# bacpop/Pansim

Measured on AMD Instinct MI355X. Metric: generations/sec, higher is better.
Workload: dtype u8

## Files before the change

pansim_amd/csrc/acc_kernels.h:

```cpp
#pragma once

#include "ps_common.h"

struct acc_dims { uint32_t N, G, W, GW; };

__global__ void acc_init_kernel(uint64_t *accG, uint64_t *accI, const uint8_t *init_vec, acc_dims d)
{
    const uint64_t t = (uint64_t)blockIdx.x * blockDim.x + threadIdx.x;
    const uint64_t nG = (uint64_t)d.G * d.W, nI = (uint64_t)d.N * d.GW;
    if (t < nG) {
        const uint32_t g = (uint32_t)(t / d.W), w = (uint32_t)(t % d.W);
        const uint32_t nb = min(64u, d.N - w * 64u);
        const uint64_t m = (nb == 64u) ? ~0ull : ((1ull << nb) - 1ull);
        accG[t] = init_vec[g] ? m : 0ull;
    } else if (t < nG + nI) {
        const uint64_t u = t - nG;
        const uint32_t gw = (uint32_t)(u % d.GW);
        uint64_t word = 0;
        for (uint32_t b = 0; b < 64; b++) {
            const uint32_t g = gw * 64u + b;
            if (g < d.G && init_vec[g]) word |= 1ull << b;
        }
        accI[u] = word;
    }
// ... 75 lines not shown
            const ps_u4 r = ps_philox(gw * 16u + j, i, a.gen, PS_STREAM_ACC_MUT, a.k0, a.k1);
            const uint4 t = thr[j];
            const uint32_t b = 4u * j;
            lt[b >> 5] |= ((r.x < t.x ? 1u : 0u) | (r.y < t.y ? 2u : 0u) | (r.z < t.z ? 4u : 0u) | (r.w < t.w ? 8u : 0u)) << (b & 31u);
        }
        word ^= ((uint64_t)lt[1] << 32) | lt[0];
    } else if (DO_MUT) {
        const uint32_t t0 = a.plan.n_comp > 0 ? a.plan.flip_thr[0] : 0u, t1 = a.plan.n_comp > 1 ? a.plan.flip_thr[1] : 0u;
        const uint64_t m0 = a.plan.n_comp > 0 ? ps_word_range_mask(gw, a.plan.comp_begin[0], a.plan.comp_end[0]) : 0ull;
        const uint64_t m1 = a.plan.n_comp > 1 ? ps_word_range_mask(gw, a.plan.comp_begin[1], a.plan.comp_end[1]) : 0ull;
        uint32_t lt0[2] = { 0u, 0u }, lt1[2] = { 0u, 0u };
#pragma unroll
        for (uint32_t j = 0; j < 16u; j++) {
            const ps_u4 r = ps_philox(gw * 16u + j, i, a.gen, PS_STREAM_ACC_MUT, a.k0, a.k1);
            const uint32_t w[4] = { r.x, r.y, r.z, r.w };
#pragma unroll
            for (uint32_t k = 0; k < 4u; k++) {
                const uint32_t b = 4u * j + k;
                lt0[b >> 5] |= (w[k] < t0 ? 1u : 0u) << (b & 31u);
                lt1[b >> 5] |= (w[k] < t1 ? 1u : 0u) << (b & 31u);
            }
        }
        const uint64_t f0 = ((uint64_t)lt0[1] << 32) | lt0[0], f1 = ((uint64_t)lt1[1] << 32) | lt1[0];
        word ^= (f1 & m1) | (f0 & m0 & ~m1);
    }
    a.dstI[t] = word;
    if (a.snapI) a.snapI[t] = word;
}

struct acc_hgt_args {
    const uint64_t *srcI;
    uint64_t *dstI;
    acc_dims d;
    uint32_t n_comp;
    uint32_t gb[PS_MAX_COMP], ge[PS_MAX_COMP];
    const uint32_t *ptab[PS_MAX_COMP];
    uint32_t kmin[PS_MAX_COMP], plen[PS_MAX_COMP];
    uint32_t *work_ctr;
    uint32_t gen, k0, k1;
    uint32_t *bins, *counts;
    uint32_t bin_cap;
    uint32_t parts, rows_per_part;
    uint32_t part_magic;
    uint32_t *scratch;
    unsigned long long *ovf_img;
    uint32_t *overflow_flag;
    uint16_t *list_scratch;
    uint32_t list_stride;
    uint32_t dn_lo, dn_cnt;
    uint32_t bin_prio;
    const uint16_t *wq[PS_MAX_COMP];
    const uint64_t *wnz[PS_MAX_COMP];
    uint32_t pref_off;
};

__device__ __forceinline__ uint32_t ps_hgt_count(const acc_hgt_args &a, uint32_t c, uint32_t dn)
{
    if (!a.ptab[c]) return 0u;
    const ps_u4 r = ps_philox(dn, 0u, a.gen, PS_STREAM_HGT_COUNT | (c << 8), a.k0, a.k1);
    uint32_t lo = 0, hi = a.plen[c];
    while (lo < hi) {
        const uint32_t mid = (lo + hi) >> 1;
        if (a.ptab[c][mid] <= r.x) lo = mid + 1u; else hi = mid;
    }
    if (lo >= a.plen[c]) lo = a.plen[c] - 1u;
    return a.kmin[c] + lo;
}

__global__ void __launch_bounds__(256) acc_snapshot_kernel(const uint64_t *copy_src, uint64_t *copy_dst, uint64_t words)
{
    for (uint64_t w = (uint64_t)blockIdx.x * blockDim.x + threadIdx.x; w < words; w += (uint64_t)gridDim.x * blockDim.x)
        copy_dst[w] = copy_src[w];
}

__device__ __forceinline__ uint32_t ps_wave_gene_list(const uint64_t *row, uint32_t GW, uint32_t gb, uint32_t ge,
                                                      uint16_t *list, uint32_t lane)
{
    uint32_t base = 0;
    for (uint32_t gw0 = gb >> 6; gw0 * 64u < ge; gw0 += 64u) {
        const uint32_t gw = gw0 + lane;
        uint64_t word = 0;
        if (gw * 64u < ge && gw < GW) {
            word = row[gw];
            const uint32_t lo = gw * 64u;
            if (lo < gb) word &= ~0ull << (gb - lo);
            if (lo + 64u > ge) word &= (ge - lo >= 64u) ? ~0ull : ((1ull << (ge - lo)) - 1ull);
        }
        const uint32_t pc = __popcll(word);
        uint32_t incl = pc;
        for (int off = 1; off < 64; off <<= 1) {
            const uint32_t t = __shfl_up(incl, off, 64);
            if ((int)lane >= off) incl += t;
        }
        uint32_t pos = base + incl - pc;
        while (word) {
            const uint32_t b = (uint32_t)__builtin_ctzll(word);
            word &= word - 1ull;
            list[pos++] = (uint16_t)(gw * 64u + b);
        }
        base += __shfl(incl, 63, 64);
    }
    return base;
}

__device__ __forceinline__ uint32_t ps_wave_gene_list_w(const uint64_t *row, uint32_t GW, uint32_t G, const uint64_t *wnz, const uint16_t *wq,
                                                        uint16_t *list, uint32_t *pref, uint32_t lane, uint32_t *total)
{
    uint32_t base = 0, wbase = 0;
    for (uint32_t gw0 = 0; gw0 * 64u < G; gw0 += 64u) {
        const uint32_t gw = gw0 + lane;
        uint64_t word = 0;
        if (gw < GW) word = row[gw] & wnz[gw];
        const uint32_t pc = __popcll(word);
        uint32_t ws = 0;
        for (uint64_t t = word; t; t &= t - 1ull) ws += wq[gw * 64u + (uint32_t)__builtin_ctzll(t)];
        uint32_t incl = pc, wincl = ws;
        for (int off = 1; off < 64; off <<= 1) {
            const uint32_t t = __shfl_up(incl, off, 64), u = __shfl_up(wincl, off, 64);
            if ((int)lane >= off) { incl += t; wincl += u; }
        }
        uint32_t pos = base + incl - pc, run = wbase + wincl - ws;
        while (word) {
            const uint32_t g = gw * 64u + (uint32_t)__builtin_ctzll(word);
            word &= word - 1ull;
            run += wq[g];
            list[pos] = (uint16_t)g;
            pref[pos++] = run;
        }
        base += __shfl(incl, 63, 64);
        wbase += __shfl(wincl, 63, 64);
    }
    *total = wbase;
    return base;
}
__device__ __forceinline__ uint32_t ps_weighted_pick(const uint32_t *pref, uint32_t n, uint32_t total, uint32_t word)
{
    const uint32_t x = ps_mulhi(word, total);
    uint32_t lo = 0, hi = n - 1u;
    while (lo < hi) {
        const uint32_t mid = (lo + hi) >> 1;
        if (pref[mid] > x) hi = mid; else lo = mid + 1u;
    }
    return lo;
}

template <bool WT = false>
__global__ void __launch_bounds__(64) acc_hgt_donor_wave_kernel(acc_hgt_args a)
{
    extern __shared__ __attribute__((aligned(16))) uint16_t lds_list[];
    uint16_t *glist = a.list_scratch ? a.list_scratch + (uint64_t)blockIdx.x * a.list_stride : lds_list;
    uint32_t *pref = (uint32_t *)(glist + a.pref_off);
    uint32_t wtotal = 0;
    const acc_dims d = a.d;
    const uint32_t lane = threadIdx.x;
    const uint32_t items = a.n_comp * a.dn_cnt;
    for (;;) {
        uint32_t item = 0;
        if (lane == 0) item = atomicAdd(a.work_ctr, 1u);
        item = __builtin_amdgcn_readfirstlane(item);
        if (item >= items) break;
        const uint32_t c = item / a.dn_cnt, dn = a.dn_lo + item % a.dn_cnt;
        const uint32_t k = ps_hgt_count(a, c, dn);
        if (k == 0u) continue;
        __threadfence_block();
        const uint32_t n = WT ? ps_wave_gene_list_w(a.srcI + (uint64_t)dn * d.GW, d.GW, d.G, a.wnz[c], a.wq[c], glist, pref, lane, &wtotal)
                              : ps_wave_gene_list(a.srcI + (uint64_t)dn * d.GW, d.GW, a.gb[c], a.ge[c], glist, lane);
        __threadfence_block();
        if (n == 0u) continue;
        const uint32_t stream = PS_STREAM_HGT | (c << 8);
        for (uint32_t jp = lane; 2u * jp < k; jp += 64u) {
            const ps_u4 r = ps_philox(jp, dn, a.gen, stream, a.k0, a.k1);
#pragma unroll
            for (uint32_t h = 0; h < 2u; h++) {
                if (2u * jp + h >= k) break;
                uint32_t rc = ps_mulhi(h ? r.z : r.x, d.N - 1u);
                rc += (rc >= dn) ? 1u : 0u;
                const uint32_t gene = glist[WT ? ps_weighted_pick(pref, n, wtotal, h ? r.w : r.y) : ps_mulhi(h ? r.w : r.y, n)];
                atomicOr((unsigned long long *)&a.dstI[(uint64_t)rc * d.GW + (gene >> 6)], 1ull << (gene & 63u));
            }
        }
    }
}

#ifndef PS_HGT_BIN_BLOCKS
#define PS_HGT_BIN_BLOCKS 2u
#endif
template <bool WT = false>
__global__ void __launch_bounds__(256) acc_hgt_donor_bin_kernel(acc_hgt_args a)
{
    extern __shared__ __attribute__((aligned(16))) uint32_t sc_lds[];
    uint32_t *fill = sc_lds;
    uint16_t *glist = a.list_scratch ? a.list_scratch + (uint64_t)blockIdx.x * a.list_stride
                                     : (uint16_t *)(sc_lds + ((a.parts + 3u) & ~3u));
    __shared__ uint32_t sh_n;
    __shared__ uint32_t sh_total;
    const uint32_t *pref = (const uint32_t *)(glist + a.pref_off);
    const acc_dims d = a.d;
    const uint32_t tid = threadIdx.x, lane = tid & 63u;
    const uint32_t items = a.n_comp * a.dn_cnt;
    const uint32_t cap = a.bin_cap;
    if (a.bin_prio >= 3u) __builtin_amdgcn_s_setprio(3);
    else if (a.bin_prio == 2u) __builtin_amdgcn_s_setprio(2);
    else if (a.bin_prio == 1u) __builtin_amdgcn_s_setprio(1);
    uint32_t *mybins = a.bins + (uint64_t)blockIdx.x * a.parts * cap;
    for (uint32_t q = tid; q < a.parts; q += blockDim.x) fill[q] = 0u;
    for (uint32_t item = blockIdx.x; item < items; item += gridDim.x) {
        __syncthreads();
        const uint32_t c = item / a.dn_cnt, dn = a.dn_lo + item % a.dn_cnt;
        const uint32_t k = ps_hgt_count(a, c, dn);
        if (k == 0u) continue;
        if (tid < 64u) {
            uint32_t tot = 0;
            const uint32_t m = WT ? ps_wave_gene_list_w(a.srcI + (uint64_t)dn * d.GW, d.GW, d.G, a.wnz[c], a.wq[c], glist, (uint32_t *)(glist + a.pref_off), lane, &tot)
                                  : ps_wave_gene_list(a.srcI + (uint64_t)dn * d.GW, d.GW, a.gb[c], a.ge[c], glist, lane);
            if (tid == 0) { sh_n = m; if (WT) sh_total = tot; }
            __threadfence_block();
        }
        __syncthreads();
        const uint32_t n = sh_n;
        if (n == 0u) continue;
        const uint32_t wtotal = WT ? sh_total : 0u;
        const uint32_t stream = PS_STREAM_HGT | (c << 8);
        auto place = [&](uint32_t rc, uint32_t gene, uint32_t part, uint32_t pos) {
            if (pos < cap) mybins[(uint64_t)part * cap + pos] = ((rc - part * a.rows_per_part) << 16) | gene;
            else atomicOr(&a.ovf_img[(uint64_t)rc * d.GW + (gene >> 6)], 1ull << (gene & 63u));
        };
        constexpr uint32_t NBK = PS_HGT_BIN_BLOCKS;
        for (uint32_t jp = tid; 2u * jp < k; jp += NBK * blockDim.x) {
            uint32_t wr[2u * NBK], wg[2u * NBK];
            bool ok[2u * NBK];
#pragma unroll
            for (uint32_t b = 0; b < NBK; b++) {
                const uint32_t jb = jp + b * blockDim.x;
                const ps_u4 r = ps_philox(jb, dn, a.gen, stream, a.k0, a.k1);
                wr[2u * b] = r.x; wg[2u * b] = r.y; wr[2u * b + 1u] = r.z; wg[2u * b + 1u] = r.w;
                ok[2u * b] = 2u * jb < k;
                ok[2u * b + 1u] = 2u * jb + 1u < k;
            }
            uint32_t rc[2u * NBK], gene[2u * NBK], part[2u * NBK], pos[2u * NBK];
#pragma unroll
            for (uint32_t e = 0; e < 2u * NBK; e++) {
                rc[e] = ps_mulhi(wr[e], d.N - 1u);
                rc[e] += (rc[e] >= dn) ? 1u : 0u;
                gene[e] = glist[WT ? ps_weighted_pick(pref, n, wtotal, wg[e]) : ps_mulhi(wg[e], n)];
                part[e] = ps_mulhi(rc[e], a.part_magic);
            }
#pragma unroll
            for (uint32_t e = 0; e < 2u * NBK; e++) pos[e] = ok[e] ? atomicAdd(&fill[part[e]], 1u) : 0u;
#pragma unroll
            for (uint32_t e = 0; e < 2u * NBK; e++)
                if (ok[e]) place(rc[e], gene[e], part[e], pos[e]);
        }
    }
    __syncthreads();
    for (uint32_t q = tid; q < a.parts; q += blockDim.x) {
        a.counts[(uint64_t)blockIdx.x * a.parts + q] = min(fill[q], cap);
    }
}

__global__ void __launch_bounds__(1024) acc_hgt_apply_kernel(acc_hgt_args a, uint32_t donor_blocks, uint32_t n_slices)
{
    extern __shared__ uint32_t lrow[];
// ... 914 lines not shown
```

pansim_amd/csrc/core_kernels.h:

```cpp
#pragma once

#include "ps_common.h"

#include <type_traits>

#define PS_SWEEP_MAX_GENS 2
struct core_sweep_args {
    uint8_t *state;
    uint8_t *out;
    const uint32_t *idx;
    const uint32_t *idx_next[PS_SWEEP_MAX_GENS - 1];
    const uint32_t *idxT;
    uint32_t N, pitch, cpr, rows;
    uint32_t site_offset;
    uint32_t gen, k0, k1;
    ps_core_plan plan;
    uint32_t *overflow_flag;
    unsigned long long *stamps;
    uint32_t *work_ctr;
    uint32_t launch_parity;
    uint32_t nt;
    uint32_t qcap;
    uint32_t qcap_limit;
    uint32_t *wide_flags;
// ... 134 lines not shown
                    const uint32_t k = ps_bit_cell(__builtin_ctz(cm));
                    cm &= cm - 1u;
                    const uint32_t i = c * 16u + k;
                    if (i >= a.N) continue;
                    uint32_t l2y;
                    const ps_cell cell = ps_cell_events<WT>(a, A, B, site, i, a.gen, a.k0, a.k1, pl, l2y);
                    if (DO_MUT && cell.mut) ps_set_byte(d, k, cell.mut);
                    if (DO_HR && cell.hr) hm |= 1u << k;
                }
            }
            if (DO_HR) {
                *(uint4 *)(rowS + 16u * c) = make_uint4(d[0], d[1], d[2], d[3]);
                hrm[c] = (uint16_t)hm;
            } else {
                *(uint4 *)(grow + 16u * c) = make_uint4(d[0], d[1], d[2], d[3]);
            }
        }
        if (DO_HR) {
            __syncthreads();
            for (uint32_t c = lane; c < a.cpr; c += lpr) {
                const uint4 v = *(const uint4 *)(rowS + 16u * c);
                uint32_t d[4] = { v.x, v.y, v.z, v.w };
                uint32_t hm = hrm[c];
                while (hm) {
                    const uint32_t k = __builtin_ctz(hm);
                    hm &= hm - 1u;
                    const uint32_t i = c * 16u + k;
                    const ps_u4 l2 = ps_philox(site, i, a.gen, PS_STREAM_CORE_L2, a.k0, a.k1);
                    uint32_t donor = ps_mulhi(l2.y, a.N - 1u);
                    donor += (donor >= i) ? 1u : 0u;
                    ps_set_byte(d, k, (uint32_t)rowS[donor]);
                }
                *(uint4 *)(grow + 16u * c) = make_uint4(d[0], d[1], d[2], d[3]);
            }
            if (!DO_GATHER) __syncthreads();
        }
    }
}

#define PS_BATCH_ROWS 4u

__device__ __forceinline__ void ps_wave_sync()
{
    __builtin_amdgcn_fence(__ATOMIC_RELEASE, "wavefront");
    __builtin_amdgcn_wave_barrier();
    __builtin_amdgcn_fence(__ATOMIC_ACQUIRE, "wavefront");
}

__device__ __forceinline__ uint32_t ps_lane_prefix(uint64_t bal)
{
    return __builtin_amdgcn_mbcnt_hi((uint32_t)(bal >> 32), __builtin_amdgcn_mbcnt_lo((uint32_t)bal, 0u));
}

__device__ __forceinline__ uint32_t ps_wave_scan_incl(uint32_t x)
{
    x += (uint32_t)__builtin_amdgcn_update_dpp(0, (int)x, 0x111, 0xF, 0xF, false);
    x += (uint32_t)__builtin_amdgcn_update_dpp(0, (int)x, 0x112, 0xF, 0xF, false);
    x += (uint32_t)__builtin_amdgcn_update_dpp(0, (int)x, 0x114, 0xF, 0xF, false);
    x += (uint32_t)__builtin_amdgcn_update_dpp(0, (int)x, 0x118, 0xF, 0xF, false);
    x += (uint32_t)__builtin_amdgcn_update_dpp(0, (int)x, 0x142, 0xA, 0xF, false);
    x += (uint32_t)__builtin_amdgcn_update_dpp(0, (int)x, 0x143, 0xC, 0xF, false);
    return x;
}

struct ps_class_words { uint32_t dec, res; };
__device__ __forceinline__ ps_class_words ps_classes(uint32_t p0, uint32_t p1, uint32_t p2, uint32_t p3, uint32_t p4, uint32_t p5,
                                                     uint32_t k, uint32_t nE, uint32_t vm)
{
    const uint32_t c1 = __builtin_amdgcn_bitop3_b32(p1, p2, p3, 0x01) & vm;
    uint32_t lt;
    switch (nE) {
    case 1: lt = __builtin_amdgcn_bitop3_b32(p0, p5, p4, 0x01); break;
    case 2: lt = __builtin_amdgcn_bitop3_b32(p0, p5, p4, 0x03); break;
    case 3: lt = __builtin_amdgcn_bitop3_b32(p0, p5, p4, 0x07); break;
    case 4: lt = __builtin_amdgcn_bitop3_b32(p0, p5, p4, 0x0F); break;
    case 5: lt = __builtin_amdgcn_bitop3_b32(p0, p5, p4, 0x1F); break;
    case 6: lt = __builtin_amdgcn_bitop3_b32(p0, p5, p4, 0x3F); break;
    case 7: lt = __builtin_amdgcn_bitop3_b32(p0, p5, p4, 0x7F); break;
    default: lt = 0xFFFFFFFFu; break;
    }
    ps_class_words o;
    o.dec = k ? c1 & __builtin_amdgcn_bitop3_b32(p0, p5, p4, 0x07) : 0u;
    o.res = c1 & lt & ~o.dec;
    return o;
}

struct ps_apply_words { uint32_t y0, y1, ya, yb, yc; };
PS_HD uint32_t ps_bfi(uint32_t m, uint32_t a, uint32_t b)
{
#if defined(__HIP_DEVICE_COMPILE__) && __has_builtin(__builtin_amdgcn_bitop3_b32)
    return __builtin_amdgcn_bitop3_b32(m, a, b, 0xCA);
#else
    return (a & m) | (b & ~m);
#endif
}
__device__ __forceinline__ ps_apply_words ps_apply_prepare(uint32_t dec, uint32_t p4, uint32_t p5)
{
    const uint32_t r1 = p5 >> 1, r2 = p4 >> 2, l1 = p5 << 1, l2 = dec << 2;
    ps_apply_words o;
    o.y0 = ps_bfi(0x01010101u, p4, ps_bfi(0x02020202u, l1, l2));
    o.y1 = ps_bfi(0x02020202u, p4, ps_bfi(0x04040404u, l1, l2));
    o.ya = ps_bfi(0x09090909u, r2, ps_bfi(0x12121212u, r1, dec));
    o.yb = ps_bfi(0x12121212u, r2, ps_bfi(0x24242424u, r1, dec));
    o.yc = ps_bfi(0x24242424u, r2, ps_bfi(0x48484848u, r1, dec));
    return o;
}
template <uint32_t SLOT>
__device__ __forceinline__ uint32_t ps_apply_dword(const ps_apply_words &y, uint32_t d)
{
    constexpr uint32_t sh = SLOT == 0u ? 0u : SLOT == 1u ? 1u : SLOT == 2u ? 0u : SLOT == 3u ? 1u : SLOT == 4u ? 2u : SLOT == 5u ? 3u : SLOT == 6u ? 4u : 5u;
    const uint32_t src = SLOT == 0u ? y.y0 : SLOT == 1u ? y.y1 : (SLOT == 2u || SLOT == 5u) ? y.ya : (SLOT == 3u || SLOT == 6u) ? y.yb : y.yc;
    const uint32_t f = (src >> sh) & 0x07070707u;
    const uint32_t allele = __builtin_amdgcn_perm(0x00080402u, 0u, f);
    const uint32_t mask = __builtin_amdgcn_perm(0x00FFFFFFu, 0u, f);
    return ps_bfi(mask, allele, d);
}
// ... 1940 lines not shown
```

pansim_amd/csrc/ps_common.h:

```cpp
#pragma once

#include <hip/hip_runtime.h>
#include <stdint.h>

#define PS_HD __host__ __device__ __forceinline__

enum : uint32_t {
    PS_STREAM_CORE_L1 = 1,
    PS_STREAM_CORE_L2 = 2,
    PS_STREAM_ACC_MUT = 3,
    PS_STREAM_HGT = 4,
    PS_STREAM_CORE_L1B = 5,
    PS_STREAM_INIT_CORE = 16,
    PS_STREAM_INIT_ACC = 17,
    PS_STREAM_SELECTION = 18,
    PS_STREAM_PAIRS = 19,
    PS_STREAM_PARENTS = 20,
    PS_STREAM_HGT_COUNT = 21
};

struct ps_u4 { uint32_t x, y, z, w; };

PS_HD uint32_t ps_mulhi(uint32_t a, uint32_t b) { return (uint32_t)(((uint64_t)a * (uint64_t)b) >> 32); }

PS_HD uint32_t ps_xor3(uint32_t a, uint32_t b, uint32_t c)
{
#if defined(__HIP_DEVICE_COMPILE__) && __has_builtin(__builtin_amdgcn_bitop3_b32)
    return __builtin_amdgcn_bitop3_b32(a, b, c, 0x96);
#else
    return a ^ b ^ c;
#endif
}

template <int ROUNDS>
PS_HD ps_u4 ps_philox_r(uint32_t c0, uint32_t c1, uint32_t c2, uint32_t c3, uint32_t k0, uint32_t k1)
{
#pragma unroll
    for (int r = 0; r < ROUNDS; r++) {
        uint64_t p0 = (uint64_t)0xD2511F53u * c0;
        uint64_t p1 = (uint64_t)0xCD9E8D57u * c2;
        uint32_t n0 = ps_xor3((uint32_t)(p1 >> 32), c1, k0);
        uint32_t n2 = ps_xor3((uint32_t)(p0 >> 32), c3, k1);
        c1 = (uint32_t)p1;
        c3 = (uint32_t)p0;
        c0 = n0;
        c2 = n2;
        k0 += 0x9E3779B9u;
        k1 += 0xBB67AE85u;
    }
    ps_u4 o = { c0, c1, c2, c3 };
    return o;
}

PS_HD ps_u4 ps_philox(uint32_t c0, uint32_t c1, uint32_t c2, uint32_t c3, uint32_t k0, uint32_t k1)
{
    return ps_philox_r<10>(c0, c1, c2, c3, k0, k1);
}

PS_HD uint32_t ps_plane_pos(uint32_t ind, uint32_t site) { return 8u * (ind & 3u) + ((ind >> 2) & 3u) + 4u * (site & 1u); }
PS_HD ps_u4 ps_philox_l1a(uint32_t site2, uint32_t chunk, uint32_t gen, uint32_t k0, uint32_t k1)
{
    return ps_philox(site2, chunk, gen, PS_STREAM_CORE_L1, k0, k1);
}
PS_HD ps_u4 ps_philox_l1b(uint32_t site4, uint32_t chunk, uint32_t gen, uint32_t k0, uint32_t k1)
{
    return ps_philox(site4, chunk, gen, PS_STREAM_CORE_L1B, k0, k1);
}

PS_HD double ps_hs_f64(uint32_t k0, uint32_t k1, uint32_t stream, uint32_t gen, uint64_t n)
{
    const uint64_t blk = n >> 1;
    const ps_u4 w = ps_philox((uint32_t)blk, (uint32_t)(blk >> 32), gen, stream, k0, k1);
    const uint64_t x = (n & 1) ? (((uint64_t)w.w << 32) | w.z) : (((uint64_t)w.y << 32) | w.x);
    return (double)(x >> 11) * (1.0 / 9007199254740992.0);
}

// ... 52 lines not shown
```

pansim_amd/csrc/pansim_capi.hip:

```cpp
#include "../../include/pansim_hip.h"

#include <hip/hip_runtime.h>

#include <algorithm>
#include <charconv>
#include <chrono>
#include <condition_variable>
#include <mutex>
#include <cmath>
#include <cstdarg>
#include <cstdio>
#include <cstdlib>
#include <cstring>
#include <string>
#include <thread>
#include <vector>

#include "acc_kernels.h"
#include "core_kernels.h"
#include "ps_common.h"

static thread_local std::string g_err;

static int ps_fail(int code, const char *fmt, ...)
// ... 1196 lines not shown
        else acc_step_rows_kernel<false, true, true><<<grid, 256, 0, st>>>(a);
    } else
    if (ga && mu) acc_step_rows_kernel<true, true><<<grid, 256, 0, st>>>(a);
    else if (ga) acc_step_rows_kernel<true, false><<<grid, 256, 0, st>>>(a);
    else acc_step_rows_kernel<false, true><<<grid, 256, 0, st>>>(a);
    HIPCHK(hipGetLastError());
    p->cur = 1 - p->cur;
    p->g_valid = false;
    p->counts_fresh = false;
    p->edit_epoch++;
    return PS_OK;
}

static int ensure_gene_major(ps_population *p, hipStream_t st)
{
    if (p->g_valid || p->d.G == 0) return PS_OK;
    acc_i_to_g_kernel<<<dim3(p->d.W, p->d.GW), 64, 0, st>>>(p->I[p->cur], p->G[0], p->d);
    HIPCHK(hipGetLastError());
    p->g_valid = true;
    return PS_OK;
}

static uint32_t hgt_partitions(const ps_population *p)
{
    const uint64_t row_bytes = (uint64_t)p->d.GW * 8;
    if (row_bytes == 0 || p->lds_limit < 1024u + row_bytes) return 0;
    const uint64_t part_cap = (p->lds_limit - 1024u) / row_bytes;
    return (uint32_t)((p->d.N + part_cap - 1) / part_cap);
}

static uint32_t hgt_pref_off(uint32_t max_comp) { return (max_comp + 7u) & ~7u; }
static uint32_t hgt_list_u16(const ps_population *p, uint32_t max_comp)
{
    return p->site_weighted ? hgt_pref_off(max_comp) + 2u * max_comp : max_comp;
}

static bool hgt_takes_binned_form(const ps_population *p)
{
    double expected = 0.0;
    uint32_t max_comp = 1;
    for (int c = 0; c < p->aplan.n_comp; c++) {
        if (p->aplan.lam_rec[c] == 0.0 || p->ptab_len[c] == 0) continue;
        expected += (double)p->d.N * p->aplan.lam_rec[c];
        max_comp = std::max(max_comp, p->aplan.comp_end[c] - p->aplan.comp_begin[c]);
    }
    const uint32_t list_lds = ((hgt_list_u16(p, max_comp) * 2u + 15u) & ~15u);
    const uint32_t parts = hgt_partitions(p);
    const uint32_t rpp = parts ? (p->d.N + parts - 1) / parts : 0;
    return parts >= 1 && parts <= 1024 && rpp >= 2 && p->d.G <= 65536u && (uint64_t)p->d.N * rpp < (1ull << 32)
           && (p->hgt_mode == 2 || (p->hgt_mode == 0 && expected >= 1.0e7))
           && list_lds + parts * 4u + 64u <= p->lds_limit;
}

static int launch_acc_hgt(ps_population *p, uint32_t gen, hipStream_t st, hipEvent_t wait_before_apply = nullptr,
                          hipEvent_t record_after_apply = nullptr, hipStream_t st_gap = nullptr, hipEvent_t ev_bin = nullptr)
{
    if (p->d.G == 0 || p->d.N < 2) return PS_OK;
    p->stream_of_call = st;
    bool counts_left = false;
    acc_hgt_args a{};
    a.n_comp = (uint32_t)p->aplan.n_comp;
    double expected = 0.0;
    uint32_t max_comp = 1;
    for (int c = 0; c < p->aplan.n_comp; c++) {
        a.gb[c] = p->aplan.comp_begin[c];
        a.ge[c] = p->aplan.comp_end[c];
        a.ptab[c] = nullptr;
        if (p->aplan.lam_rec[c] == 0.0 || p->ptab_len[c] == 0) continue;
        a.ptab[c] = p->d_ptab[c];
        a.kmin[c] = p->ptab_kmin[c];
        a.plen[c] = p->ptab_len[c];
        expected += (double)p->d.N * p->aplan.lam_rec[c];
        max_comp = std::max(max_comp, a.ge[c] - a.gb[c]);
    }
    if (expected == 0.0) return PS_OK;
    a.d = p->d;
    a.gen = gen;
    a.k0 = (uint32_t)p->cfg.seed;
    a.k1 = (uint32_t)(p->cfg.seed >> 32);
    a.work_ctr = p->cnt + (uint64_t)PS_MAX_COMP * p->d.N;
    a.overflow_flag = p->d_flag;
    const bool sharded = p->donor_cnt != 0;
    a.dn_lo = sharded ? p->donor_lo : 0u;
    a.dn_cnt = sharded ? p->donor_cnt : p->d.N;
    const uint32_t items = a.n_comp * a.dn_cnt;
    const uint64_t mat_words = (uint64_t)p->d.N * p->d.GW;
    if (sharded && !p->d_delta) {
        p->delta_words = (mat_words + 4095) & ~4095ull;
        HIPCHK(hipMalloc(&p->d_delta, p->delta_words * 8));
        HIPCHK(hipMemsetAsync(p->d_delta, 0, p->delta_words * 8, st));
    }
    const bool wt = p->site_weighted;
    if (wt) {
        const uint64_t GW = p->d.GW, G64 = GW * 64;
        const uint8_t *nz = p->d_gene_tab + G64 * 4, *wq = nz + (uint64_t)PS_MAX_COMP * GW * 8;
        for (int c = 0; c < p->aplan.n_comp; c++) {
            a.wnz[c] = (const uint64_t *)nz + (uint64_t)c * GW;
            a.wq[c] = (const uint16_t *)wq + (uint64_t)c * G64;
        }
        a.pref_off = hgt_pref_off(max_comp);
    }
    const uint32_t list_u16 = hgt_list_u16(p, max_comp);
    const uint32_t list_lds = ((list_u16 * 2u + 15u) & ~15u);
    if (list_lds > p->lds_limit)
        return ps_fail(PS_ERR_INVALID, "a compartment of %u genes needs %u bytes of LDS (limit %u)", max_comp, list_lds, p->lds_limit);

// ... 57 lines not shown
        if (dlds > 64 * 1024)
            HIPCHK(hipFuncSetAttribute((const void *)bin_kern, hipFuncAttributeMaxDynamicSharedMemorySize, (int)dlds));
        hipLaunchKernelGGL(bin_kern, dim3(donor_blocks), dim3(256), dlds, st, a);
        const bool in_gap = st_gap && ev_bin && record_after_apply && !p->exchange_beside_sweep;
        hipStream_t run = st;
        if (in_gap) {
            HIPCHK(hipEventRecord(ev_bin, st));
            HIPCHK(hipStreamWaitEvent(st_gap, ev_bin, 0));
            run = st_gap;
        } else if (wait_before_apply) HIPCHK(hipStreamWaitEvent(st, wait_before_apply, 0));
        auto kern = acc_hgt_apply_kernel;
        if (lds > 64 * 1024)
            HIPCHK(hipFuncSetAttribute((const void *)kern, hipFuncAttributeMaxDynamicSharedMemorySize, (int)lds));
        hipLaunchKernelGGL(kern, dim3(parts * n_slices), dim3(p->hgt_apply_threads), lds, run, a, donor_blocks, n_slices);
        if (record_after_apply && (!sharded || p->exchange_beside_sweep)) {
            HIPCHK(hipEventRecord(record_after_apply, run));
            if (in_gap) HIPCHK(hipStreamWaitEvent(st, record_after_apply, 0));
            record_after_apply = nullptr;
            run = st;
        }
        st = run;
        if (!sharded && p->fuse_counts_out) {
            acc_hgt_reduce_rows_kernel<<<(uint32_t)((p->d.N + 3) / 4), 256, 0, st>>>((const uint64_t *)p->hgt_scratch, p->I[p->cur], p->d,
                                                                                    n_slices, (unsigned long long *)p->hgt_ovf_img,
                                                                                    p->fuse_counts_out, p->fuse_logw_out);
            counts_left = true;
        } else
        acc_hgt_reduce_kernel<<<(uint32_t)((words + 255) / 256), 256, 0, st>>>((const uint64_t *)p->hgt_scratch,
                                                                              sharded ? p->d_delta : p->I[p->cur], words, n_slices,
                                                                              sharded ? 1 : 0, (unsigned long long *)p->hgt_ovf_img);
    } else {
        a.srcI = have_snapshot ? p->I_snap : p->I[1 - p->cur];
        a.dstI = sharded ? p->d_delta : p->I[p->cur];
        if (sharded) HIPCHK(hipMemsetAsync(p->d_delta, 0, mat_words * 8, st));
        uint32_t grid = std::min(items, 256u * 32u);
        if (p->hgt_events_per_thread) {
            const double expected_here = expected * (double)a.dn_cnt / (double)p->d.N;
            const uint64_t want = (uint64_t)(expected_here / ((double)p->hgt_events_per_thread * 64.0)) + 1;
            grid = (uint32_t)std::min<uint64_t>(std::max<uint64_t>(want, 1), grid);
        }
        uint32_t dyn_lds = list_lds;
        if (p->hgt_list_in_global) {
            const uint64_t need = (uint64_t)grid * list_u16 * sizeof(uint16_t);
            if (p->hgt_scratch_cap < need) {
                if (p->hgt_scratch) HIPCHK(hipFree(p->hgt_scratch));
                p->hgt_scratch = nullptr;
                p->hgt_scratch_cap = 0;
                HIPCHK(hipMalloc(&p->hgt_scratch, need));
                p->hgt_scratch_cap = need;
            }
            a.list_scratch = (uint16_t *)p->hgt_scratch;
            a.list_stride = list_u16;
            dyn_lds = 0;
        }
        auto wave_kern = wt ? acc_hgt_donor_wave_kernel<true> : acc_hgt_donor_wave_kernel<false>;
        if (dyn_lds > 64 * 1024)
            HIPCHK(hipFuncSetAttribute((const void *)wave_kern, hipFuncAttributeMaxDynamicSharedMemorySize, (int)dyn_lds));
        hipLaunchKernelGGL(wave_kern, dim3(grid), dim3(64), dyn_lds, st, a);
    }
    HIPCHK(hipGetLastError());
    if (sharded) {
        if (p->exchange) {
            const std::string prev = g_err;
            g_err.clear();
            const int rc = p->exchange(p->exchange_ctx, p->d_delta, p->delta_words, (void *)st);
            if (rc != 0) {
                const std::string inner = g_err;
                return ps_fail(PS_ERR_STATE, "the HGT delta exchange failed (%d)%s%s", rc, inner.empty() ? "" : ": ", inner.c_str());
            }
            g_err = prev;
        }
        if (p->fuse_counts_out) {
            acc_or_rows_kernel<<<(uint32_t)((p->d.N + 3) / 4), 256, 0, st>>>(p->I[p->cur], p->d_delta, p->d, p->fuse_counts_out, p->fuse_logw_out);
            counts_left = true;
        } else
        acc_or_kernel<<<(uint32_t)((mat_words + 255) / 256), 256, 0, st>>>(p->I[p->cur], p->d_delta, mat_words);
        HIPCHK(hipGetLastError());
    }
    if (record_after_apply) {
        HIPCHK(hipEventRecord(record_after_apply, st));
        if (st != p->stream_of_call) HIPCHK(hipStreamWaitEvent(p->stream_of_call, record_after_apply, 0));
    }
    p->g_valid = false;
    p->counts_fresh = counts_left;
    p->edit_epoch++;
    return PS_OK;
}

extern "C" int ps_set_donor_shard(ps_population *p, uint32_t shard_rank, uint32_t shard_count, ps_exchange_fn fn, void *ctx)
{
    if (!p) return ps_fail(PS_ERR_INVALID, "null handle");
    if (p->cfg.core) return ps_fail(PS_ERR_INVALID, "donor shards apply to the accessory matrix (HGT, population.rs:544-751)");
    if (shard_count < 1 || shard_rank >= shard_count) return ps_fail(PS_ERR_INVALID, "bad donor shard %u of %u", shard_rank, shard_count);
    const uint64_t N = p->cfg.pop_size;
    if (shard_count == 1) {
        p->donor_lo = 0;
        p->donor_cnt = 0;
        p->exchange = nullptr;
        p->exchange_ctx = nullptr;
        return PS_OK;
    }
    const uint64_t lo = N * shard_rank / shard_count, hi = N * ((uint64_t)shard_rank + 1) / shard_count;
    if (hi <= lo) return ps_fail(PS_ERR_INVALID, "more donor shards than individuals");
    p->donor_lo = (uint32_t)lo;
    p->donor_cnt = (uint32_t)(hi - lo);
    p->exchange = fn;
    p->exchange_ctx = ctx;
// ... 2872 lines not shown
```

Baseline: 3073.

## Wave-parallelize HGT count search, use DPP scans, batch donor atomics

```diff
diff --git a/pansim_amd/csrc/acc_kernels.h b/pansim_amd/csrc/acc_kernels.h
--- a/pansim_amd/csrc/acc_kernels.h
+++ b/pansim_amd/csrc/acc_kernels.h
@@ -153,16 +153,35 @@
     uint32_t pref_off;
 };
 
-__device__ __forceinline__ uint32_t ps_hgt_count(const acc_hgt_args &a, uint32_t c, uint32_t dn)
+#ifndef PS_HGT_WAVE_PROLOGUE
+#define PS_HGT_WAVE_PROLOGUE 1
+#endif
+__device__ __forceinline__ uint32_t ps_hgt_count(const acc_hgt_args &a, uint32_t c, uint32_t dn, uint32_t lane)
 {
     if (!a.ptab[c]) return 0u;
     const ps_u4 r = ps_philox(dn, 0u, a.gen, PS_STREAM_HGT_COUNT | (c << 8), a.k0, a.k1);
-    uint32_t lo = 0, hi = a.plen[c];
-    while (lo < hi) {
-        const uint32_t mid = (lo + hi) >> 1;
-        if (a.ptab[c][mid] <= r.x) lo = mid + 1u; else hi = mid;
-    }
-    if (lo >= a.plen[c]) lo = a.plen[c] - 1u;
+    const uint32_t *thr = a.ptab[c];
+    const uint32_t plen = a.plen[c];
+    uint32_t lo;
+    if (PS_HGT_WAVE_PROLOGUE && plen <= 4096u) {
+        const uint32_t stride = (plen + 63u) >> 6;
+        const uint32_t end = min(lane * stride + stride, plen);
+        const bool whole = lane * stride < plen && thr[end - 1u] <= r.x;
+        lo = min((uint32_t)__popcll(__ballot(whole)) * stride, plen);
+        if (stride > 1u && lo < plen) {
+            const uint32_t idx = lo + lane;
+            const bool le = lane < stride && idx < plen && thr[min(idx, plen - 1u)] <= r.x;
+            lo += (uint32_t)__popcll(__ballot(le));
+        }
+    } else {
+        uint32_t hi = plen;
+        lo = 0;
+        while (lo < hi) {
+            const uint32_t mid = (lo + hi) >> 1;
+            if (thr[mid] <= r.x) lo = mid + 1u; else hi = mid;
+        }
+    }
+    if (lo >= plen) lo = plen - 1u;
     return a.kmin[c] + lo;
 }
 
@@ -187,6 +206,8 @@
         }
         const uint32_t pc = __popcll(word);
         uint32_t incl = pc;
+        if (PS_HGT_WAVE_PROLOGUE) incl = ps_wave_scan_incl(pc);
+        else
         for (int off = 1; off < 64; off <<= 1) {
             const uint32_t t = __shfl_up(incl, off, 64);
             if ((int)lane >= off) incl += t;
@@ -197,7 +218,7 @@
             word &= word - 1ull;
             list[pos++] = (uint16_t)(gw * 64u + b);
         }
-        base += __shfl(incl, 63, 64);
+        base += (uint32_t)__builtin_amdgcn_readlane((int)incl, 63);
     }
     return base;
 }
@@ -214,6 +235,8 @@
         uint32_t ws = 0;
         for (uint64_t t = word; t; t &= t - 1ull) ws += wq[gw * 64u + (uint32_t)__builtin_ctzll(t)];
         uint32_t incl = pc, wincl = ws;
+        if (PS_HGT_WAVE_PROLOGUE) { incl = ps_wave_scan_incl(pc); wincl = ps_wave_scan_incl(ws); }
+        else
         for (int off = 1; off < 64; off <<= 1) {
             const uint32_t t = __shfl_up(incl, off, 64), u = __shfl_up(wincl, off, 64);
             if ((int)lane >= off) { incl += t; wincl += u; }
@@ -226,8 +249,8 @@
             list[pos] = (uint16_t)g;
             pref[pos++] = run;
         }
-        base += __shfl(incl, 63, 64);
-        wbase += __shfl(wincl, 63, 64);
+        base += (uint32_t)__builtin_amdgcn_readlane((int)incl, 63);
+        wbase += (uint32_t)__builtin_amdgcn_readlane((int)wincl, 63);
     }
     *total = wbase;
     return base;
@@ -243,6 +266,9 @@
     return lo;
 }
 
+#ifndef PS_HGT_WAVE_BLOCKS
+#define PS_HGT_WAVE_BLOCKS 2u
+#endif
 template <bool WT = false>
 __global__ void __launch_bounds__(64) acc_hgt_donor_wave_kernel(acc_hgt_args a)
 {
@@ -259,7 +285,7 @@
         item = __builtin_amdgcn_readfirstlane(item);
         if (item >= items) break;
         const uint32_t c = item / a.dn_cnt, dn = a.dn_lo + item % a.dn_cnt;
-        const uint32_t k = ps_hgt_count(a, c, dn);
+        const uint32_t k = ps_hgt_count(a, c, dn, lane);
         if (k == 0u) continue;
         __threadfence_block();
         const uint32_t n = WT ? ps_wave_gene_list_w(a.srcI + (uint64_t)dn * d.GW, d.GW, d.G, a.wnz[c], a.wq[c], glist, pref, lane, &wtotal)
@@ -267,16 +293,30 @@
         __threadfence_block();
         if (n == 0u) continue;
         const uint32_t stream = PS_STREAM_HGT | (c << 8);
-        for (uint32_t jp = lane; 2u * jp < k; jp += 64u) {
-            const ps_u4 r = ps_philox(jp, dn, a.gen, stream, a.k0, a.k1);
-#pragma unroll
-            for (uint32_t h = 0; h < 2u; h++) {
-                if (2u * jp + h >= k) break;
-                uint32_t rc = ps_mulhi(h ? r.z : r.x, d.N - 1u);
-                rc += (rc >= dn) ? 1u : 0u;
-                const uint32_t gene = glist[WT ? ps_weighted_pick(pref, n, wtotal, h ? r.w : r.y) : ps_mulhi(h ? r.w : r.y, n)];
-                atomicOr((unsigned long long *)&a.dstI[(uint64_t)rc * d.GW + (gene >> 6)], 1ull << (gene & 63u));
-            }
+        constexpr uint32_t NBK = PS_HGT_WAVE_BLOCKS;
+        for (uint32_t jp = lane; 2u * jp < k; jp += NBK * 64u) {
+            uint32_t wr[2u * NBK], wg[2u * NBK];
+            bool ok[2u * NBK];
+#pragma unroll
+            for (uint32_t b = 0; b < NBK; b++) {
+                const uint32_t jb = jp + b * 64u;
+                const ps_u4 r = ps_philox(jb, dn, a.gen, stream, a.k0, a.k1);
+                wr[2u * b] = r.x; wg[2u * b] = r.y; wr[2u * b + 1u] = r.z; wg[2u * b + 1u] = r.w;
+                ok[2u * b] = 2u * jb < k;
+                ok[2u * b + 1u] = 2u * jb + 1u < k;
+            }
+            uint32_t rc[2u * NBK], at[2u * NBK], gene[2u * NBK];
+#pragma unroll
+            for (uint32_t e = 0; e < 2u * NBK; e++) {
+                rc[e] = ps_mulhi(wr[e], d.N - 1u);
+                rc[e] += (rc[e] >= dn) ? 1u : 0u;
+                at[e] = !ok[e] ? 0u : WT ? ps_weighted_pick(pref, n, wtotal, wg[e]) : ps_mulhi(wg[e], n);
+            }
+#pragma unroll
+            for (uint32_t e = 0; e < 2u * NBK; e++) gene[e] = glist[at[e]];
+#pragma unroll
+            for (uint32_t e = 0; e < 2u * NBK; e++)
+                if (ok[e]) atomicOr((unsigned long long *)&a.dstI[(uint64_t)rc[e] * d.GW + (gene[e] >> 6)], 1ull << (gene[e] & 63u));
         }
     }
 }
@@ -306,7 +346,7 @@
     for (uint32_t item = blockIdx.x; item < items; item += gridDim.x) {
         __syncthreads();
         const uint32_t c = item / a.dn_cnt, dn = a.dn_lo + item % a.dn_cnt;
-        const uint32_t k = ps_hgt_count(a, c, dn);
+        const uint32_t k = ps_hgt_count(a, c, dn, lane);
         if (k == 0u) continue;
         if (tid < 64u) {
             uint32_t tot = 0;
diff --git a/pansim_amd/csrc/core_kernels.h b/pansim_amd/csrc/core_kernels.h
--- a/pansim_amd/csrc/core_kernels.h
+++ b/pansim_amd/csrc/core_kernels.h
@@ -210,16 +210,6 @@
     return __builtin_amdgcn_mbcnt_hi((uint32_t)(bal >> 32), __builtin_amdgcn_mbcnt_lo((uint32_t)bal, 0u));
 }
 
-__device__ __forceinline__ uint32_t ps_wave_scan_incl(uint32_t x)
-{
-    x += (uint32_t)__builtin_amdgcn_update_dpp(0, (int)x, 0x111, 0xF, 0xF, false);
-    x += (uint32_t)__builtin_amdgcn_update_dpp(0, (int)x, 0x112, 0xF, 0xF, false);
-    x += (uint32_t)__builtin_amdgcn_update_dpp(0, (int)x, 0x114, 0xF, 0xF, false);
-    x += (uint32_t)__builtin_amdgcn_update_dpp(0, (int)x, 0x118, 0xF, 0xF, false);
-    x += (uint32_t)__builtin_amdgcn_update_dpp(0, (int)x, 0x142, 0xA, 0xF, false);
-    x += (uint32_t)__builtin_amdgcn_update_dpp(0, (int)x, 0x143, 0xC, 0xF, false);
-    return x;
-}
 
 struct ps_class_words { uint32_t dec, res; };
 __device__ __forceinline__ ps_class_words ps_classes(uint32_t p0, uint32_t p1, uint32_t p2, uint32_t p3, uint32_t p4, uint32_t p5,
diff --git a/pansim_amd/csrc/ps_common.h b/pansim_amd/csrc/ps_common.h
--- a/pansim_amd/csrc/ps_common.h
+++ b/pansim_amd/csrc/ps_common.h
@@ -22,6 +22,17 @@
 struct ps_u4 { uint32_t x, y, z, w; };
 
 PS_HD uint32_t ps_mulhi(uint32_t a, uint32_t b) { return (uint32_t)(((uint64_t)a * (uint64_t)b) >> 32); }
+
+__device__ __forceinline__ uint32_t ps_wave_scan_incl(uint32_t x)
+{
+    x += (uint32_t)__builtin_amdgcn_update_dpp(0, (int)x, 0x111, 0xF, 0xF, false);
+    x += (uint32_t)__builtin_amdgcn_update_dpp(0, (int)x, 0x112, 0xF, 0xF, false);
+    x += (uint32_t)__builtin_amdgcn_update_dpp(0, (int)x, 0x114, 0xF, 0xF, false);
+    x += (uint32_t)__builtin_amdgcn_update_dpp(0, (int)x, 0x118, 0xF, 0xF, false);
+    x += (uint32_t)__builtin_amdgcn_update_dpp(0, (int)x, 0x142, 0xA, 0xF, false);
+    x += (uint32_t)__builtin_amdgcn_update_dpp(0, (int)x, 0x143, 0xC, 0xF, false);
+    return x;
+}
 
 PS_HD uint32_t ps_xor3(uint32_t a, uint32_t b, uint32_t c)
 {
```

Result: slower. 2769 (-9.9%).

## Pipeline HGT wave kernel: prefetch next item, stage threshold tables in LDS

Applied to the files above, without the earlier changes.

```diff
diff --git a/pansim_amd/csrc/acc_kernels.h b/pansim_amd/csrc/acc_kernels.h
--- a/pansim_amd/csrc/acc_kernels.h
+++ b/pansim_amd/csrc/acc_kernels.h
@@ -151,6 +151,9 @@
     const uint16_t *wq[PS_MAX_COMP];
     const uint64_t *wnz[PS_MAX_COMP];
     uint32_t pref_off;
+    uint32_t tab_lds_off;
+    uint32_t tab_off[PS_MAX_COMP];
+    unsigned long long *stamps;
 };
 
 __device__ __forceinline__ uint32_t ps_hgt_count(const acc_hgt_args &a, uint32_t c, uint32_t dn)
@@ -172,62 +175,76 @@
         copy_dst[w] = copy_src[w];
 }
 
+__device__ __forceinline__ uint32_t ps_gene_list_chunk(uint64_t word, uint32_t gw, uint32_t gb, uint32_t ge, uint16_t *list, uint32_t lane, uint32_t base)
+{
+    const uint32_t lo = gw * 64u;
+    if (lo < gb) word &= ~0ull << (gb - lo);
+    if (lo + 64u > ge) word &= (ge - lo >= 64u) ? ~0ull : ((1ull << (ge - lo)) - 1ull);
+    const uint32_t pc = __popcll(word);
+    uint32_t incl = pc;
+    for (int off = 1; off < 64; off <<= 1) {
+        const uint32_t t = __shfl_up(incl, off, 64);
+        if ((int)lane >= off) incl += t;
+    }
+    uint32_t pos = base + incl - pc;
+    while (word) {
+        const uint32_t b = (uint32_t)__builtin_ctzll(word);
+        word &= word - 1ull;
+        list[pos++] = (uint16_t)(gw * 64u + b);
+    }
+    return base + __shfl(incl, 63, 64);
+}
 __device__ __forceinline__ uint32_t ps_wave_gene_list(const uint64_t *row, uint32_t GW, uint32_t gb, uint32_t ge,
-                                                      uint16_t *list, uint32_t lane)
-{
-    uint32_t base = 0;
-    for (uint32_t gw0 = gb >> 6; gw0 * 64u < ge; gw0 += 64u) {
+                                                      uint16_t *list, uint32_t lane, bool have_first = false, uint64_t first = 0)
+{
+    uint32_t base = 0, gw0 = gb >> 6;
+    if (have_first) {
+        if (gw0 * 64u < ge) base = ps_gene_list_chunk(first, gw0 + lane, gb, ge, list, lane, base);
+        gw0 += 64u;
+    }
+    for (; gw0 * 64u < ge; gw0 += 64u) {
         const uint32_t gw = gw0 + lane;
-        uint64_t word = 0;
-        if (gw * 64u < ge && gw < GW) {
-            word = row[gw];
-            const uint32_t lo = gw * 64u;
-            if (lo < gb) word &= ~0ull << (gb - lo);
-            if (lo + 64u > ge) word &= (ge - lo >= 64u) ? ~0ull : ((1ull << (ge - lo)) - 1ull);
-        }
-        const uint32_t pc = __popcll(word);
-        uint32_t incl = pc;
-        for (int off = 1; off < 64; off <<= 1) {
-            const uint32_t t = __shfl_up(incl, off, 64);
-            if ((int)lane >= off) incl += t;
-        }
-        uint32_t pos = base + incl - pc;
-        while (word) {
-            const uint32_t b = (uint32_t)__builtin_ctzll(word);
-            word &= word - 1ull;
-            list[pos++] = (uint16_t)(gw * 64u + b);
-        }
-        base += __shfl(incl, 63, 64);
+        const uint64_t word = (gw * 64u < ge && gw < GW) ? row[gw] : 0ull;
+        base = ps_gene_list_chunk(word, gw, gb, ge, list, lane, base);
     }
     return base;
 }
 
+__device__ __forceinline__ void ps_gene_list_chunk_w(uint64_t word, uint32_t gw, const uint16_t *wq, uint16_t *list, uint32_t *pref, uint32_t lane,
+                                                     uint32_t *base, uint32_t *wbase)
+{
+    const uint32_t pc = __popcll(word);
+    uint32_t ws = 0;
+    for (uint64_t t = word; t; t &= t - 1ull) ws += wq[gw * 64u + (uint32_t)__builtin_ctzll(t)];
+    uint32_t incl = pc, wincl = ws;
+    for (int off = 1; off < 64; off <<= 1) {
+        const uint32_t t = __shfl_up(incl, off, 64), u = __shfl_up(wincl, off, 64);
+        if ((int)lane >= off) { incl += t; wincl += u; }
+    }
+    uint32_t pos = *base + incl - pc, run = *wbase + wincl - ws;
+    while (word) {
+        const uint32_t g = gw * 64u + (uint32_t)__builtin_ctzll(word);
+        word &= word - 1ull;
+        run += wq[g];
+        list[pos] = (uint16_t)g;
+        pref[pos++] = run;
+    }
+    *base += __shfl(incl, 63, 64);
+    *wbase += __shfl(wincl, 63, 64);
+}
 __device__ __forceinline__ uint32_t ps_wave_gene_list_w(const uint64_t *row, uint32_t GW, uint32_t G, const uint64_t *wnz, const uint16_t *wq,
-                                                        uint16_t *list, uint32_t *pref, uint32_t lane, uint32_t *total)
-{
-    uint32_t base = 0, wbase = 0;
-    for (uint32_t gw0 = 0; gw0 * 64u < G; gw0 += 64u) {
+                                                        uint16_t *list, uint32_t *pref, uint32_t lane, uint32_t *total,
+                                                        bool have_first = false, uint64_t first = 0)
+{
+    uint32_t base = 0, wbase = 0, gw0 = 0;
+    if (have_first) {
+        if (G > 0u) ps_gene_list_chunk_w(lane < GW ? first & wnz[lane] : 0ull, lane, wq, list, pref, lane, &base, &wbase);
+        gw0 = 64u;
+    }
+    for (; gw0 * 64u < G; gw0 += 64u) {
         const uint32_t gw = gw0 + lane;
-        uint64_t word = 0;
-        if (gw < GW) word = row[gw] & wnz[gw];
-        const uint32_t pc = __popcll(word);
-        uint32_t ws = 0;
-        for (uint64_t t = word; t; t &= t - 1ull) ws += wq[gw * 64u + (uint32_t)__builtin_ctzll(t)];
-        uint32_t incl = pc, wincl = ws;
-        for (int off = 1; off < 64; off <<= 1) {
-            const uint32_t t = __shfl_up(incl, off, 64), u = __shfl_up(wincl, off, 64);
-            if ((int)lane >= off) { incl += t; wincl += u; }
-        }
-        uint32_t pos = base + incl - pc, run = wbase + wincl - ws;
-        while (word) {
-            const uint32_t g = gw * 64u + (uint32_t)__builtin_ctzll(word);
-            word &= word - 1ull;
-            run += wq[g];
-            list[pos] = (uint16_t)g;
-            pref[pos++] = run;
-        }
-        base += __shfl(incl, 63, 64);
-        wbase += __shfl(wincl, 63, 64);
+        const uint64_t word = gw < GW ? row[gw] & wnz[gw] : 0ull;
+        ps_gene_list_chunk_w(word, gw, wq, list, pref, lane, &base, &wbase);
     }
     *total = wbase;
     return base;
@@ -243,42 +260,152 @@
     return lo;
 }
 
+#ifdef PS_HGT_STAMP
+#define PS_HT(k) do { unsigned long long t_; asm volatile("s_waitcnt lgkmcnt(0)\n\ts_memrealtime %0\n\ts_waitcnt lgkmcnt(0)" : "=s"(t_) :: "memory"); ht_acc[k] += t_ - ht_last; ht_last = t_; } while (0)
+#else
+#define PS_HT(k) do { } while (0)
+#endif
+
+__device__ __forceinline__ uint32_t ps_threshold_rank(const uint32_t *tab, uint32_t plen, uint32_t x)
+{
+    uint32_t lo = 0, hi = plen;
+    while (lo < hi) {
+        const uint32_t mid = (lo + hi) >> 1;
+        if (tab[mid] <= x) lo = mid + 1u; else hi = mid;
+    }
+    return lo >= plen ? plen - 1u : lo;
+}
+
+template <bool WT>
+__device__ __forceinline__ uint64_t ps_hgt_first_word(const acc_hgt_args &a, uint32_t c, uint32_t dn, uint32_t lane)
+{
+    const uint32_t gw = (WT ? 0u : a.gb[c] >> 6) + lane;
+    const bool in = WT ? gw < a.d.GW : (gw * 64u < a.ge[c] && gw < a.d.GW);
+    return in ? a.srcI[(uint64_t)dn * a.d.GW + gw] : 0ull;
+}
+
+__device__ __forceinline__ void ps_weighted_pick4(const uint32_t *pref, uint32_t n, uint32_t total, const uint32_t word[4], uint32_t out[4])
+{
+    uint32_t x[4], lo[4], hi[4];
+#pragma unroll
+    for (uint32_t e = 0; e < 4u; e++) { x[e] = ps_mulhi(word[e], total); lo[e] = 0u; hi[e] = n - 1u; }
+    const uint32_t steps = n > 1u ? 32u - (uint32_t)__builtin_clz(n - 1u) : 0u;
+    for (uint32_t s = 0; s < steps; s++) {
+        uint32_t mid[4], v[4];
+#pragma unroll
+        for (uint32_t e = 0; e < 4u; e++) { mid[e] = (lo[e] + hi[e]) >> 1; v[e] = pref[mid[e]]; }
+#pragma unroll
+        for (uint32_t e = 0; e < 4u; e++)
+            if (lo[e] < hi[e]) { if (v[e] > x[e]) hi[e] = mid[e]; else lo[e] = mid[e] + 1u; }
+    }
+#pragma unroll
+    for (uint32_t e = 0; e < 4u; e++) out[e] = lo[e];
+}
+
+template <bool WT, bool GL>
+__device__ __forceinline__ void ps_hgt_donor_wave(const acc_hgt_args &a, uint16_t *glist, uint32_t *ltab, const uint32_t lane)
+{
+    uint32_t *pref = (uint32_t *)(glist + a.pref_off);
+    const acc_dims d = a.d;
+    const uint32_t items = a.n_comp * a.dn_cnt;
+#ifdef PS_HGT_STAMP
+    unsigned long long ht_acc[4] = { 0, 0, 0, 0 };
+    unsigned long long ht_last, ht_first;
+    asm volatile("s_memrealtime %0\n\ts_waitcnt lgkmcnt(0)" : "=s"(ht_last) :: "memory");
+    ht_first = ht_last;
+#endif
+    auto list_fence = [&]() {
+        if (GL) __threadfence_block();
+        else __builtin_amdgcn_fence(__ATOMIC_SEQ_CST, "wavefront");
+    };
+    uint32_t grab = 0;
+    if (lane == 0) grab = atomicAdd(a.work_ctr, 1u);
+    if (!GL && ltab) {
+        for (uint32_t c = 0; c < a.n_comp; c++) {
+            if (!a.ptab[c]) continue;
+            for (uint32_t q = lane; q < a.plen[c]; q += 64u) ltab[a.tab_off[c] + q] = a.ptab[c][q];
+        }
+        list_fence();
+    }
+    PS_HT(0);
+    uint32_t n_item = 0, n_c = 0, n_dn = 0, n_k = 0;
+    uint64_t n_word = 0;
+    bool n_live = false;
+    auto count_stage = [&]() {
+        n_item = __builtin_amdgcn_readfirstlane(grab);
+        n_live = n_item < items;
+        n_k = 0u;
+        n_word = 0ull;
+        if (!n_live) return;
+        n_c = n_item / a.dn_cnt;
+        n_dn = a.dn_lo + n_item % a.dn_cnt;
+        if (a.ptab[n_c]) {
+            const ps_u4 r = ps_philox(n_dn, 0u, a.gen, PS_STREAM_HGT_COUNT | (n_c << 8), a.k0, a.k1);
+            const uint32_t rank = (!GL && ltab) ? ps_threshold_rank(ltab + a.tab_off[n_c], a.plen[n_c], r.x)
+                                                : ps_threshold_rank(a.ptab[n_c], a.plen[n_c], r.x);
+            n_k = a.kmin[n_c] + rank;
+        }
+        if (n_k) n_word = ps_hgt_first_word<WT>(a, n_c, n_dn, lane);
+        if (lane == 0) grab = atomicAdd(a.work_ctr, 1u);
+    };
+    count_stage();
+    PS_HT(1);
+    while (n_live) {
+        const uint32_t c = n_c, dn = n_dn, k = n_k;
+        const uint64_t word = n_word;
+        count_stage();
+        PS_HT(1);
+        if (k == 0u) continue;
+        uint32_t wtotal = 0;
+        list_fence();
+        const uint32_t n = WT ? ps_wave_gene_list_w(a.srcI + (uint64_t)dn * d.GW, d.GW, d.G, a.wnz[c], a.wq[c], glist, pref, lane, &wtotal, true, word)
+                              : ps_wave_gene_list(a.srcI + (uint64_t)dn * d.GW, d.GW, a.gb[c], a.ge[c], glist, lane, true, word);
+        list_fence();
+        PS_HT(2);
+        if (n == 0u) continue;
+        const uint32_t stream = PS_STREAM_HGT | (c << 8);
+        for (uint32_t jb = 0; 2u * jb < k; jb += 128u) {
+            const uint32_t jp = jb + lane;
+            const ps_u4 r0 = ps_philox(jp, dn, a.gen, stream, a.k0, a.k1);
+            ps_u4 r1 = { 0u, 0u, 0u, 0u };
+            if (2u * (jb + 64u) < k) r1 = ps_philox(jp + 64u, dn, a.gen, stream, a.k0, a.k1);
+            const uint32_t wr[4] = { r0.x, r0.z, r1.x, r1.z }, wg[4] = { r0.y, r0.w, r1.y, r1.w };
+            const bool ok[4] = { 2u * jp < k, 2u * jp + 1u < k, 2u * (jp + 64u) < k, 2u * (jp + 64u) + 1u < k };
+            uint32_t rc[4], pick[4], gene[4];
+#pragma unroll
+            for (uint32_t e = 0; e < 4u; e++) {
+                rc[e] = ps_mulhi(wr[e], d.N - 1u);
+                rc[e] += (rc[e] >= dn) ? 1u : 0u;
+            }
+            if (WT) ps_weighted_pick4(pref, n, wtotal, wg, pick);
+            else {
+#pragma unroll
+                for (uint32_t e = 0; e < 4u; e++) pick[e] = ps_mulhi(wg[e], n);
+            }
+#pragma unroll
+            for (uint32_t e = 0; e < 4u; e++) gene[e] = glist[pick[e]];
+#pragma unroll
+            for (uint32_t e = 0; e < 4u; e++)
+                if (ok[e]) atomicOr((unsigned long long *)&a.dstI[(uint64_t)rc[e] * d.GW + (gene[e] >> 6)], 1ull << (gene[e] & 63u));
+        }
+        PS_HT(3);
+    }
+#ifdef PS_HGT_STAMP
+    if (lane == 0) {
+        for (int q = 0; q < 4; q++) atomicAdd(a.stamps + q, ht_acc[q]);
+        atomicAdd(a.stamps + 4, 1ull);
+        atomicAdd(a.stamps + 5, ht_last - ht_first);
+    }
+#endif
+}
+
 template <bool WT = false>
 __global__ void __launch_bounds__(64) acc_hgt_donor_wave_kernel(acc_hgt_args a)
 {
     extern __shared__ __attribute__((aligned(16))) uint16_t lds_list[];
-    uint16_t *glist = a.list_scratch ? a.list_scratch + (uint64_t)blockIdx.x * a.list_stride : lds_list;
-    uint32_t *pref = (uint32_t *)(glist + a.pref_off);
-    uint32_t wtotal = 0;
-    const acc_dims d = a.d;
     const uint32_t lane = threadIdx.x;
-    const uint32_t items = a.n_comp * a.dn_cnt;
-    for (;;) {
-        uint32_t item = 0;
-        if (lane == 0) item = atomicAdd(a.work_ctr, 1u);
-        item = __builtin_amdgcn_readfirstlane(item);
-        if (item >= items) break;
-        const uint32_t c = item / a.dn_cnt, dn = a.dn_lo + item % a.dn_cnt;
-        const uint32_t k = ps_hgt_count(a, c, dn);
-        if (k == 0u) continue;
-        __threadfence_block();
-        const uint32_t n = WT ? ps_wave_gene_list_w(a.srcI + (uint64_t)dn * d.GW, d.GW, d.G, a.wnz[c], a.wq[c], glist, pref, lane, &wtotal)
-                              : ps_wave_gene_list(a.srcI + (uint64_t)dn * d.GW, d.GW, a.gb[c], a.ge[c], glist, lane);
-        __threadfence_block();
-        if (n == 0u) continue;
-        const uint32_t stream = PS_STREAM_HGT | (c << 8);
-        for (uint32_t jp = lane; 2u * jp < k; jp += 64u) {
-            const ps_u4 r = ps_philox(jp, dn, a.gen, stream, a.k0, a.k1);
-#pragma unroll
-            for (uint32_t h = 0; h < 2u; h++) {
-                if (2u * jp + h >= k) break;
-                uint32_t rc = ps_mulhi(h ? r.z : r.x, d.N - 1u);
-                rc += (rc >= dn) ? 1u : 0u;
-                const uint32_t gene = glist[WT ? ps_weighted_pick(pref, n, wtotal, h ? r.w : r.y) : ps_mulhi(h ? r.w : r.y, n)];
-                atomicOr((unsigned long long *)&a.dstI[(uint64_t)rc * d.GW + (gene >> 6)], 1ull << (gene & 63u));
-            }
-        }
-    }
+    if (a.list_scratch) ps_hgt_donor_wave<WT, true>(a, a.list_scratch + (uint64_t)blockIdx.x * a.list_stride, nullptr, lane);
+    else ps_hgt_donor_wave<WT, false>(a, lds_list, a.tab_lds_off ? (uint32_t *)((uint8_t *)lds_list + a.tab_lds_off) : nullptr, lane);
 }
 
 #ifndef PS_HGT_BIN_BLOCKS
diff --git a/pansim_amd/csrc/pansim_capi.hip b/pansim_amd/csrc/pansim_capi.hip
--- a/pansim_amd/csrc/pansim_capi.hip
+++ b/pansim_amd/csrc/pansim_capi.hip
@@ -1272,6 +1272,7 @@
            && list_lds + parts * 4u + 64u <= p->lds_limit;
 }
 
+#define PS_HGT_WAVE_LDS_BUDGET (16u * 1024u)
 static int launch_acc_hgt(ps_population *p, uint32_t gen, hipStream_t st, hipEvent_t wait_before_apply = nullptr,
                           hipEvent_t record_after_apply = nullptr, hipStream_t st_gap = nullptr, hipEvent_t ev_bin = nullptr)
 {
@@ -1435,7 +1436,17 @@
             a.list_scratch = (uint16_t *)p->hgt_scratch;
             a.list_stride = list_u16;
             dyn_lds = 0;
-        }
+        } else {
+            uint32_t tab_u32 = 0;
+            for (uint32_t c = 0; c < a.n_comp; c++)
+                if (a.ptab[c]) { a.tab_off[c] = tab_u32; tab_u32 += a.plen[c]; }
+            const uint64_t with_tables = (uint64_t)list_lds + (((uint64_t)tab_u32 * 4u + 15u) & ~15ull);
+            if (with_tables <= std::min<uint64_t>(PS_HGT_WAVE_LDS_BUDGET, p->lds_limit)) {
+                a.tab_lds_off = list_lds;
+                dyn_lds = (uint32_t)with_tables;
+            }
+        }
+        a.stamps = p->d_stamps;
         auto wave_kern = wt ? acc_hgt_donor_wave_kernel<true> : acc_hgt_donor_wave_kernel<false>;
         if (dyn_lds > 64 * 1024)
             HIPCHK(hipFuncSetAttribute((const void *)wave_kern, hipFuncAttributeMaxDynamicSharedMemorySize, (int)dyn_lds));
```

Result: slower. 3075 before, 2797 after (-9.0%).
